# probabilists/zuko

Hardware: AMD Instinct MI355X
Metric: log_prob samples/sec, NSF d=64 K=8 bins=8 batch=2^20 (higher is better)
Workload: dtype f32; 1 GPU; NSF(features=64, context=0, transforms=8, bins=8, hidden=[256]*3) log_prob, batch=2^20 per GPU, x~N(0,1), seed-0 init; batch_per_gpu=1048576, global_batch=1048576, parallelism=batch-sharded x1, one RCCL all-reduce of the scalar NLL

## Files before the change

zuko_amd/csrc/fused_ar_half_impl.h:

```cpp
#pragma once
#include "fused_ar_split_impl.h"

#ifndef ARH_LOOK
#define ARH_LOOK 1
#endif
#ifndef ARH_RELU_INT
#define ARH_RELU_INT 0
#endif
#ifndef ARH_EPI_PINNED
#define ARH_EPI_PINNED 1
#endif
#ifndef ARH_DESCALE_PK
#define ARH_DESCALE_PK 1
#endif
#ifndef ARH_PREFETCH
#define ARH_PREFETCH 1
#endif
#ifndef ARH_BLOCK_ASM
#define ARH_BLOCK_ASM 1
#endif
#ifndef ARH_EPI_TILE
#define ARH_EPI_TILE 1
#endif

#ifndef ARH_SPLIT_GAPS
#define ARH_SPLIT_GAPS 1
#endif

namespace zk {

typedef _Float16 f16x8 __attribute__((ext_vector_type(8)));

struct ArhB {
  f16x8 h, l;
};

__device__ __forceinline__ void arh_scale(float& amax, float& s, float& inv_s) {
  amax = fmaxf(amax, __shfl_xor(amax, 16, 64));
  amax = fmaxf(amax, __shfl_xor(amax, 32, 64));
  int e = __builtin_amdgcn_frexp_expf(amax);
  int ea = 15 - e;
  ea = ea > 90 ? 90 : (ea < -90 ? -90 : ea);
  s = __builtin_amdgcn_ldexpf(1.0f, ea);
  inv_s = __builtin_amdgcn_ldexpf(1.0f, -ea);
}

#define ARH_AMAX_OVERFLOW (65520.f * 0x1p90f)

typedef unsigned arh_u32x4 __attribute__((ext_vector_type(4)));
typedef float arh_f32x2 __attribute__((ext_vector_type(2)));

__device__ __forceinline__ void arh_split(const f32x4& lo, const f32x4& hi, float s, ArhB& b) {
  if (ARX_ABL == 6) {
    b.h = __builtin_bit_cast(f16x8, lo); b.l = __builtin_bit_cast(f16x8, hi);
    return;
  }
#if ARH_EPI_PINNED
  const float nz = -0.f;
  unsigned h0, h1, h2, h3, l0, l1, l2, l3;
#define ARH_SPLIT_H(OP, H, V) "v_fma_mix" OP "_f16 %[" H "], %[" V "], %[s], %[nz]\n\t"
#define ARH_SPLIT_L(OP, SEL, L, H, V) "v_fma_mix" OP "_f16 %[" L "], %[" V "], %[s], -%[" H "] op_sel:[0,0," SEL "] op_sel_hi:[0,0,1]\n\t"
  asm(ARH_SPLIT_H("lo", "h0", "v0") ARH_SPLIT_H("lo", "h1", "v2") ARH_SPLIT_H("lo", "h2", "v4") ARH_SPLIT_H("lo", "h3", "v6")
      ARH_SPLIT_H("hi", "h0", "v1") ARH_SPLIT_H("hi", "h1", "v3") ARH_SPLIT_H("hi", "h2", "v5") ARH_SPLIT_H("hi", "h3", "v7")
      ARH_SPLIT_L("lo", "0", "l0", "h0", "v0") ARH_SPLIT_L("lo", "0", "l1", "h1", "v2") ARH_SPLIT_L("lo", "0", "l2", "h2", "v4") ARH_SPLIT_L("lo", "0", "l3", "h3", "v6")
      ARH_SPLIT_L("hi", "1", "l0", "h0", "v1") ARH_SPLIT_L("hi", "1", "l1", "h1", "v3") ARH_SPLIT_L("hi", "1", "l2", "h2", "v5") ARH_SPLIT_L("hi", "1", "l3", "h3", "v7")
      : [h0] "=&v"(h0), [h1] "=&v"(h1), [h2] "=&v"(h2), [h3] "=&v"(h3), [l0] "=&v"(l0), [l1] "=&v"(l1), [l2] "=&v"(l2), [l3] "=&v"(l3)
      : [v0] "v"(lo[0]), [v1] "v"(lo[1]), [v2] "v"(lo[2]), [v3] "v"(lo[3]), [v4] "v"(hi[0]), [v5] "v"(hi[1]), [v6] "v"(hi[2]), [v7] "v"(hi[3]), [s] "v"(s), [nz] "s"(nz));
#undef ARH_SPLIT_H
#undef ARH_SPLIT_L
  b.h = __builtin_bit_cast(f16x8, arh_u32x4{h0, h1, h2, h3}); b.l = __builtin_bit_cast(f16x8, arh_u32x4{l0, l1, l2, l3});
  return;
#endif
#pragma unroll
  for (int e = 0; e < 8; ++e) {
    const float v = (e < 4 ? lo[e] : hi[e - 4]) * s;
    const _Float16 h = (_Float16)v;
    const float r = v - (float)h;
    b.h[e] = h;
    b.l[e] = (_Float16)r;
  }
}

#define ARH_MFMA(A, B, C) C = __builtin_amdgcn_mfma_f32_16x16x32_f16(__builtin_bit_cast(f16x8, A), B, C, 0, 0, 0)
__device__ __forceinline__ void arh_block(const f32x4 (&a)[2], const ArhB& b, f32x4& c) {
  if (ARX_ABL == 2) {
    asm volatile("" ::"v"(a[0]), "v"(a[1]));
    return;
  }
  ARH_MFMA(a[1], b.h, c);
  ARH_MFMA(a[0], b.l, c);
  ARH_MFMA(a[0], b.h, c);
}

__device__ __forceinline__ void arh_touch(f32x4& v) { asm volatile("" : "+v"(v)); }
template <int N> __device__ __forceinline__ void arh_settle(f32x4& a0, f32x4& a1) { asm volatile("s_waitcnt lgkmcnt(%2)" : "+v"(a0), "+v"(a1) : "n"(N)); }
template <int N> __device__ __forceinline__ void arh_settle(f32x4& a0, f32x4& a1, f32x4& a2) { asm volatile("s_waitcnt lgkmcnt(%3)" : "+v"(a0), "+v"(a1), "+v"(a2) : "n"(N)); }

constexpr bool ARH_BLK = ARH_BLOCK_ASM && ARX_ABL != 2;
constexpr bool ARH_GAPS = ARH_SPLIT_GAPS && ARH_BLK && ARH_EPI_PINNED && ARX_ABL != 6;
struct ArhHL {
  unsigned h0, h1, h2, h3, l0, l1, l2, l3;
};
#define ARH_GH(OP, H, V) "\n\tv_fma_mix" OP "_f16 %[" H "], %[" V "], %[s], %[nz]"
#define ARH_GL(OP, SEL, L, H, V) "\n\tv_fma_mix" OP "_f16 %[" L "], %[" V "], %[s], -%[" H "] op_sel:[0,0," SEL "] op_sel_hi:[0,0,1]"
#define ARH_G0 ARH_GH("lo", "h0", "v0")
#define ARH_G1 ARH_GH("lo", "h1", "v2")
#define ARH_G2 ARH_GH("lo", "h2", "v4")
#define ARH_G3 ARH_GH("lo", "h3", "v6")
#define ARH_G4 ARH_GH("hi", "h0", "v1")
#define ARH_G5 ARH_GH("hi", "h1", "v3")
#define ARH_G6 ARH_GH("hi", "h2", "v5")
#define ARH_G7 ARH_GH("hi", "h3", "v7")
#define ARH_G8 ARH_GL("lo", "0", "l0", "h0", "v0")
#define ARH_G9 ARH_GL("lo", "0", "l1", "h1", "v2")
#define ARH_G10 ARH_GL("lo", "0", "l2", "h2", "v4")
#define ARH_G11 ARH_GL("lo", "0", "l3", "h3", "v6")
#define ARH_G12 ARH_GL("hi", "1", "l0", "h0", "v1")
#define ARH_G13 ARH_GL("hi", "1", "l1", "h1", "v3")
#define ARH_G14 ARH_GL("hi", "1", "l2", "h2", "v5")
#define ARH_G15 ARH_GL("hi", "1", "l3", "h3", "v7")
#define ARH_G_OUT0
#define ARH_G_IN0
#define ARH_G_SC [s] "v"(s), [nz] "s"(nz)
#define ARH_G_OUT1 , [h0] "=&v"(x.h0), [l0] "=&v"(x.l0)
#define ARH_G_IN1 , [v0] "v"(lo[0]), [v1] "v"(lo[1]), ARH_G_SC
#define ARH_G_OUT2 , [l0] "+v"(x.l0), [h1] "=&v"(x.h1)
#define ARH_G_IN2 , [v1] "v"(lo[1]), [h0] "v"(x.h0), [v2] "v"(lo[2]), [v3] "v"(lo[3]), ARH_G_SC
#define ARH_G_OUT3 , [l1] "=&v"(x.l1), [h2] "=&v"(x.h2)
#define ARH_G_IN3 , [v2] "v"(lo[2]), [v3] "v"(lo[3]), [h1] "v"(x.h1), [v4] "v"(hi[0]), ARH_G_SC
#define ARH_G_OUT4 , [h2] "+v"(x.h2), [l2] "=&v"(x.l2)
#define ARH_G_IN4 , [v5] "v"(hi[1]), [v4] "v"(hi[0]), ARH_G_SC
#define ARH_G_OUT5 , [h3] "=&v"(x.h3), [l3] "=&v"(x.l3)
#define ARH_G_IN5 , [v6] "v"(hi[2]), [v7] "v"(hi[3]), ARH_G_SC
#define ARH_G_OUT6 , [l3] "+v"(x.l3)
#define ARH_G_IN6 , [v7] "v"(hi[3]), [h3] "v"(x.h3), [s] "v"(s)
#define ARH_T_OUT2 [l0] "+v"(x.l0), [h1] "=&v"(x.h1), [l1] "=&v"(x.l1), [h2] "=&v"(x.h2), [l2] "=&v"(x.l2), [h3] "=&v"(x.h3), [l3] "=&v"(x.l3)
#define ARH_T_IN2 [v1] "v"(lo[1]), [v2] "v"(lo[2]), [v3] "v"(lo[3]), [v4] "v"(hi[0]), [v5] "v"(hi[1]), [v6] "v"(hi[2]), [v7] "v"(hi[3]), [h0] "v"(x.h0), ARH_G_SC
#define ARH_T_OUT3 [l1] "=&v"(x.l1), [h2] "=&v"(x.h2), [l2] "=&v"(x.l2), [h3] "=&v"(x.h3), [l3] "=&v"(x.l3)
#define ARH_T_IN3 [v2] "v"(lo[2]), [v3] "v"(lo[3]), [v4] "v"(hi[0]), [v5] "v"(hi[1]), [v6] "v"(hi[2]), [v7] "v"(hi[3]), [h1] "v"(x.h1), ARH_G_SC
#define ARH_T_OUT4 [h2] "+v"(x.h2), [l2] "=&v"(x.l2), [h3] "=&v"(x.h3), [l3] "=&v"(x.l3)
#define ARH_T_IN4 [v4] "v"(hi[0]), [v5] "v"(hi[1]), [v6] "v"(hi[2]), [v7] "v"(hi[3]), ARH_G_SC
#define ARH_T_OUT5 [h3] "=&v"(x.h3), [l3] "=&v"(x.l3)
#define ARH_T_IN5 [v6] "v"(hi[2]), [v7] "v"(hi[3]), ARH_G_SC
#define ARH_T_OUT6 [l3] "+v"(x.l3)
#define ARH_T_IN6 [v7] "v"(hi[3]), [h3] "v"(x.h3), [s] "v"(s)
#define ARH_BLK_ASM(C0, COUT, POST, BSOUT, G1, G2, G3, G)                                                   \
  asm volatile("v_mfma_f32_16x16x32_f16 %[c], %[al], %[bh], " C0 G1 "\n\t"                                  \
               "v_mfma_f32_16x16x32_f16 %[c], %[ah], %[bl], %[c]" G2 "\n\t"                                 \
               "v_mfma_f32_16x16x32_f16 %[c], %[ah], %[bh], %[c]" G3 POST                                   \
               : [c] COUT(c) ARH_BLK_BS##BSOUT ARH_G_OUT##G                                                 \
               : [ah] "v"(a[0]), [al] "v"(a[1]), [bh] "v"(b.h), [bl] "v"(b.l) ARH_G_IN##G)
#define ARH_BLK_BS0
#define ARH_BLK_BS1 , "+v"(bs)
#define ARH_BLK_FORM(G1, G2, G3, G)                                                               \
  if constexpr (FIRST && TILE) ARH_BLK_ASM("0", "=&v", "\n\ts_nop 11", 1, G1, G2, G3, G);          \
  else if constexpr (FIRST) ARH_BLK_ASM("0", "=&v", "", 0, G1, G2, G3, G);                         \
  else if constexpr (TILE) ARH_BLK_ASM("%[c]", "+v", "\n\ts_nop 11", 1, G1, G2, G3, G);            \
  else ARH_BLK_ASM("%[c]", "+v", "", 0, G1, G2, G3, G)
template <int N, bool FIRST, bool PAD, bool TILE> __device__ __forceinline__ void arh_wait_block(f32x4 (&a)[2], const ArhB& b, f32x4& c, f32x4& bs) {
  static_assert(N >= 0 && N < 16, "lgkmcnt is a four-bit field");
  if constexpr (PAD) asm volatile("s_nop 0");
  __builtin_amdgcn_s_waitcnt(0xC07F | (N << 8));
  if (ARX_FENCE) __builtin_amdgcn_sched_barrier(0);
  ARH_BLK_FORM("", "", "", 0);
  if (ARX_FENCE) __builtin_amdgcn_sched_barrier(0);
}
template <int N, bool FIRST, bool PAD, bool TILE, int GF>
__device__ __forceinline__ void arh_wait_block(f32x4 (&a)[2], const ArhB& b, f32x4& c, f32x4& bs, ArhHL& x, const f32x4& lo, const f32x4& hi, float s) {
  static_assert(N >= 0 && N < 16 && GF >= 1 && GF <= 6, "lgkmcnt is a four-bit field; six forms");
  const float nz = -0.f;
  if constexpr (PAD) asm volatile("s_nop 0");
  __builtin_amdgcn_s_waitcnt(0xC07F | (N << 8));
  if (ARX_FENCE) __builtin_amdgcn_sched_barrier(0);
  if constexpr (GF == 1) { ARH_BLK_FORM(ARH_G0, ARH_G4, ARH_G8, 1); }
  else if constexpr (GF == 2) { ARH_BLK_FORM(ARH_G12, ARH_G1, ARH_G5, 2); }
  else if constexpr (GF == 3) { ARH_BLK_FORM(ARH_G9, ARH_G13, ARH_G2, 3); }
  else if constexpr (GF == 4) { ARH_BLK_FORM(ARH_G6, ARH_G10, ARH_G14, 4); }
  else if constexpr (GF == 5) { ARH_BLK_FORM(ARH_G3, ARH_G7, ARH_G11, 5); }
  else { ARH_BLK_FORM(ARH_G15, "", "", 6); }
  if (ARX_FENCE) __builtin_amdgcn_sched_barrier(0);
}
template <int F> __device__ __forceinline__ void arh_split_tail(ArhHL& x, const f32x4& lo, const f32x4& hi, float s) {
  static_assert(F >= 2 && F <= 6, "six forms");
  const float nz = -0.f;
#define ARH_T6 ARH_G15
#define ARH_T5 ARH_G3 ARH_G7 ARH_G11 ARH_T6
#define ARH_T4 ARH_G6 ARH_G10 ARH_G14 ARH_T5
#define ARH_T3 ARH_G9 ARH_G13 ARH_G2 ARH_T4
#define ARH_T2 ARH_G12 ARH_G1 ARH_G5 ARH_T3
#define ARH_TAIL_ASM(T, F) asm("; the rest of a split" T : ARH_T_OUT##F : ARH_T_IN##F)
  if constexpr (F == 2) ARH_TAIL_ASM(ARH_T2, 2);
  else if constexpr (F == 3) ARH_TAIL_ASM(ARH_T3, 3);
  else if constexpr (F == 4) ARH_TAIL_ASM(ARH_T4, 4);
  else if constexpr (F == 5) ARH_TAIL_ASM(ARH_T5, 5);
  else ARH_TAIL_ASM(ARH_T6, 6);
#undef ARH_TAIL_ASM
#undef ARH_T2
#undef ARH_T3
#undef ARH_T4
#undef ARH_T5
#undef ARH_T6
}
__device__ __forceinline__ void arh_split_done(const ArhHL& x, ArhB& b) {
  b.h = __builtin_bit_cast(f16x8, arh_u32x4{x.h0, x.h1, x.h2, x.h3}); b.l = __builtin_bit_cast(f16x8, arh_u32x4{x.l0, x.l1, x.l2, x.l3});
  asm volatile("" : "+v"(b.h), "+v"(b.l));
}
#undef ARH_BLK_FORM
#undef ARH_BLK_ASM
#undef ARH_BLK_BS0
#undef ARH_BLK_BS1
#undef ARH_G_OUT0
#undef ARH_G_IN0
#undef ARH_G_OUT1
#undef ARH_G_IN1
#undef ARH_G_OUT2
#undef ARH_G_IN2
#undef ARH_G_OUT3
#undef ARH_G_IN3
#undef ARH_G_OUT4
#undef ARH_G_IN4
#undef ARH_G_OUT5
#undef ARH_G_IN5
#undef ARH_G_OUT6
#undef ARH_G_IN6
#undef ARH_G_SC
#undef ARH_T_OUT2
#undef ARH_T_IN2
#undef ARH_T_OUT3
#undef ARH_T_IN3
#undef ARH_T_OUT4
#undef ARH_T_IN4
#undef ARH_T_OUT5
#undef ARH_T_IN5
#undef ARH_T_OUT6
#undef ARH_T_IN6
#undef ARH_GH
#undef ARH_GL
#undef ARH_G0
#undef ARH_G1
#undef ARH_G2
#undef ARH_G3
#undef ARH_G4
#undef ARH_G5
#undef ARH_G6
#undef ARH_G7
#undef ARH_G8
#undef ARH_G9
#undef ARH_G10
#undef ARH_G11
#undef ARH_G12
#undef ARH_G13
#undef ARH_G14
#undef ARH_G15
template <int NT> __device__ __forceinline__ void arh_acc_ready(f32x4 (&acc)[NT]) {
  asm volatile("s_nop 11" : "+v"(acc[NT - 1]));
#pragma unroll
  for (int t = 0; t + 1 < NT; ++t) arh_touch(acc[t]);
}

__device__ __forceinline__ void arh_relu_max(f32x4& o, float (&pm)[4], int t) {
#pragma unroll
  for (int r = 0; r < 4; r += 2)
    asm("v_max_f32 %0, 0, %0\n\tv_max_f32 %1, 0, %1\n\tv_max3_f32 %2, %2, %0, %1" : "+v"(o[r]), "+v"(o[r + 1]), "+v"(pm[(2 * t + r / 2) % 4]));
}
__device__ __forceinline__ float arh_join_max(const float (&pm)[4]) {
  float amax;
  asm("v_max_f32 %0, %1, %2\n\tv_max3_f32 %0, %0, %3, %4" : "=&v"(amax) : "v"(pm[0]), "v"(pm[1]), "v"(pm[2]), "v"(pm[3]));
  return amax;
}

template <int WAVES, int CH, int NR> struct ArhRing : ArRingS<WAVES, CH, NR> {
  typedef ArRingS<WAVES, CH, NR> B;
  template <int XV> __device__ __forceinline__ void advance_x() {
    asm volatile("s_waitcnt vmcnt(%0) lgkmcnt(0)" ::"n"((NR - 2) * B::PER + XV) : "memory");
    if (ARX_ABL != 4) __builtin_amdgcn_s_barrier();
    asm volatile("" ::: "memory");
    this->issue();
    this->slot = (this->slot + 1 == NR) ? 0 : this->slot + 1;
    this->cur_off = this->lds_off + (unsigned)(this->slot * CH * AR_TF * 4 + this->lane * 16);
  }
  template <int S, int XV = 0> __device__ __forceinline__ f32x4 read() {
    if constexpr (XV != 0 && S % CH == 0) {
      advance_x<XV>();
      f32x4 v;
      if (ARX_ABL == 5) {
        asm volatile("v_mov_b32 %0, %1" : "=v"(v[0]) : "v"(this->cur_off));
        v[1] = v[2] = v[3] = v[0];
        return v;
      }
      asm volatile("ds_read_b128 %0, %1 offset:%2" : "=v"(v) : "v"(this->cur_off), "n"((S % CH) * AR_TF * 4));
      return v;
    } else {
      return B::template read<S>();
    }
  }
};

template <int WAVES, int CH, int IMAGES, int BPOS, bool FLOW = false> struct ArhRing4 {
  static constexpr int NR = 4, PER = CH / WAVES, PIVOT = PER > 4 ? 4 : 0, CHB = CH * AR_TF * 4, NCH = (IMAGES + CH - 1) / CH;
  static_assert(PER * WAVES == CH && PER <= 6 && BPOS % 2 == 0 && BPOS >= 2 * (ARH_LOOK + 1) && BPOS + 1 < CH && CH % 2 == 0 && IMAGES % 2 == 0, "ring geometry");
  static constexpr int trigger(int c) {
    const int last = (IMAGES < (c + 1) * CH ? IMAGES : (c + 1) * CH) - 1;
    return c * CH + BPOS + 1 < last ? c * CH + BPOS + 1 : last;
  }
  static constexpr int first_trigger_from(int pos) {
    for (int c = 0; c < NCH; ++c)
      if (trigger(c) >= pos) return trigger(c);
    return -1;
  }
  const char* gsrc;
  char* ldst;
  unsigned goff, gend;
  unsigned fill_off;
  unsigned read_off;
  unsigned lane_off;
  unsigned lane16;
  unsigned cur_off;
  bool rows_in_flight;
  const char* bias_src;
  char* bias_dst;
  int bias_n, wave_id;
  __device__ __forceinline__ void bias_request() {
    for (int p = wave_id; p < bias_n; p += WAVES)
      __builtin_amdgcn_global_load_lds((const __attribute__((address_space(1))) void*)(bias_src + p * 1024 + (size_t)lane16), (__attribute__((address_space(3))) void*)(bias_dst + p * 1024), 16, 0, 0);
  }
  __device__ __forceinline__ void start(float* lds, const float* stream, int n_chunks, int wave, int lane) {
    const int b0 = wave * PER + PIVOT;
    gsrc = reinterpret_cast<const char*>(stream + b0 * AR_TF);
    ldst = reinterpret_cast<char*>(lds + b0 * AR_TF);
    goff = 0; gend = (unsigned)n_chunks * CHB; fill_off = 0;
    lane16 = (unsigned)lane * 16;
    lane_off = (unsigned)(size_t)((__attribute__((address_space(3))) float*)lds) + lane16;
    if constexpr (FLOW) { wave_id = wave; rows_in_flight = false; bias_n = 0; }
#pragma unroll
    for (int i = 0; i < NR - 1; ++i) issue();
    read_off = (NR - 1) * CHB;
    cur_off = lane_off;
  }
  template <int I> __device__ __forceinline__ void dma(const char* g, char* l) {
    if constexpr (I < PER) {
      __builtin_amdgcn_global_load_lds((const __attribute__((address_space(1))) void*)g, (__attribute__((address_space(3))) void*)l, 16, (I - PIVOT) * AR_TF * 4, 0);
      dma<I + 1>(g, l);
    }
  }
  __device__ __forceinline__ void issue() {
    asm volatile("" : "+v"(lane16));
    if (ARX_ABL != 1) dma<0>(gsrc + goff + (size_t)lane16, ldst + fill_off);
    goff = (goff + CHB == gend) ? 0 : goff + CHB;
    fill_off = (fill_off + CHB == NR * CHB) ? 0 : fill_off + CHB;
  }
  template <int XV, bool DRAIN> __device__ __forceinline__ void wait() {
    if constexpr (DRAIN) asm volatile("s_waitcnt vmcnt(%0) lgkmcnt(0)" ::"n"(XV) : "memory");
    else asm volatile("s_waitcnt vmcnt(%0)" ::"n"(XV) : "memory");
  }
  template <int XV, bool DRAIN> __device__ __forceinline__ void boundary() {
    if constexpr (FLOW && XV != 0) {
      if (rows_in_flight) wait<XV, DRAIN>();
      else wait<0, DRAIN>();
    } else {
      wait<XV, DRAIN>();
    }
    if (ARX_ABL != 4) __builtin_amdgcn_s_barrier();
    asm volatile("" ::: "memory");
    issue();
    asm volatile("" ::: "memory");
  }
  template <int S, int XV = 0> __device__ __forceinline__ f32x4 read() {
    static_assert(S >= 0 && S < IMAGES, "stream position");
    if constexpr (S % CH == 0) {
      read_off = (read_off + CHB == NR * CHB) ? 0 : read_off + CHB;
      cur_off = lane_off + read_off;
    }
    f32x4 v;
    if (ARX_ABL == 5) {
      asm volatile("v_mov_b32 %0, %1" : "=v"(v[0]) : "v"(cur_off));
      v[1] = v[2] = v[3] = v[0];
    } else {
      asm volatile("ds_read_b128 %0, %1 offset:%2" : "=v"(v) : "v"(cur_off), "n"((S % CH) * AR_TF * 4));
    }
    if constexpr (S == trigger(S / CH)) boundary<XV, (S % CH != BPOS + 1)>();
    if constexpr (FLOW && NCH >= 2) {
      if constexpr (S == trigger(NCH - 2)) bias_request();
    }
    return v;
  }
};

template <class S, int L, bool ALT> constexpr int arh_ip(int s) {
  if constexpr (ALT) return S::B_IP_ALT[s];
  else return ArxPat<S>::ip(L, s);
}
template <class S> constexpr bool ARH_EPI = S::ACT == 1 && ARH_EPI_PINNED && ARH_EPI_TILE;

template <int NBLK> struct ArhGapPlan {
  signed char pair[NBLK > 0 ? NBLK : 1], form[NBLK > 0 ? NBLK : 1];
  short lim[9];
  signed char front[9];
};
template <class S, int L, int NT> constexpr int arh_gap_blocks() {
  if constexpr (L == S::NH) return S::GOFF[S::NG] * NT;
  else return S::NB[L];
}
template <class S, int L, int NT> constexpr int arh_gap_reader(int b) {
  if constexpr (L == S::NH) return S::G_IP[b / NT];
  else return ArxPat<S>::ip(L, b);
}
template <class S, int L> constexpr int arh_gap_last_block(int t) {
  if (t >= S::HT[L]) return S::NB[L];
  int last = -1;
  for (int b = 0; b < S::NB[L]; ++b)
    if (ArxPat<S>::ot(L, b) == t) last = b;
  return last;
}
template <class S, int L, int NT> constexpr ArhGapPlan<arh_gap_blocks<S, L, NT>()> arh_gap_plan() {
  static_assert(L >= 1 && L <= S::NH && S::TMAX / 2 <= 8, "a consuming layer; eight in pairs at most");
  constexpr int NBLK = arh_gap_blocks<S, L, NT>(), NP = (S::HT[L - 1] + 1) / 2;
  ArhGapPlan<NBLK> g{};
  for (int p = 0; p < 9; ++p) { g.lim[p] = 0; g.front[p] = 7; }
  int cursor = 0;
  for (int p = 1; p < NP; ++p) {
    int lim = NBLK;
    for (int b = NBLK - 1; b >= 0; --b)
      if (arh_gap_reader<S, L, NT>(b) == p) lim = b;
    if constexpr (L != S::NH) {
      for (int t = 2 * p; t <= 2 * p + 1; ++t) {
        const int last = arh_gap_last_block<S, L>(t);
        lim = last < 0 ? 0 : (last < lim ? last : lim);
      }
    }
    int f = 1;
    for (; f <= 6 && cursor < lim; ++f, ++cursor) { g.pair[cursor] = (signed char)p; g.form[cursor] = (signed char)f; }
    g.lim[p] = (short)lim;
    g.front[p] = (signed char)f;
  }
  return g;
}
template <class S, int L, int NT, bool ON> struct ArhGapsOf {
  static constexpr int NP = 0, NBLK = 0;
  static constexpr int form(int) { return 0; }
  static constexpr int pair(int) { return 0; }
  static constexpr bool tail_at(int, int) { return false; }
  static constexpr bool any_tail_at(int) { return false; }
  static constexpr int front(int) { return 7; }
};
template <class S, int L, int NT> struct ArhGapsOf<S, L, NT, true> {
  static constexpr int NP = (S::HT[L - 1] + 1) / 2, NBLK = arh_gap_blocks<S, L, NT>();
  static constexpr ArhGapPlan<NBLK> plan = arh_gap_plan<S, L, NT>();
  static constexpr int form(int b) { return plan.form[b]; }
  static constexpr int pair(int b) { return plan.pair[b]; }
  static constexpr bool tail_at(int p, int b) { return p >= 1 && plan.front[p] <= 6 && plan.lim[p] == b; }
  static constexpr int front(int p) { return plan.front[p]; }
  static constexpr bool any_tail_at(int b) {
    for (int p = 1; p < NP; ++p)
      if (tail_at(p, b)) return true;
    return false;
  }
};
template <class GP, int HTI, int NPR> __device__ __forceinline__ void arh_gap_front(const f32x4 (&out)[2 * NPR], float s, ArhB (&in)[NPR]) {
  const f32x4 zero = {0.f, 0.f, 0.f, 0.f};
  arh_split(out[0], 1 < HTI ? out[1] : zero, s, in[0]);
  ars_for<GP::NP>([&](auto p_) ARS_ALWAYS_INLINE {
    constexpr int p = p_;
    if constexpr (GP::tail_at(p, 0)) arh_split(out[2 * p], 2 * p + 1 < HTI ? out[2 * p + 1] : zero, s, in[p]);
  });
}
template <class GP, int HTI, int B, int NPR> __device__ __forceinline__ void arh_gap_tails(ArhHL (&x)[NPR], const f32x4 (&out)[2 * NPR], float s, ArhB (&in)[NPR]) {
  const f32x4 zero = {0.f, 0.f, 0.f, 0.f};
  ars_for<GP::NP>([&](auto p_) ARS_ALWAYS_INLINE {
    constexpr int p = p_;
    if constexpr (B >= 1 && GP::tail_at(p, B)) {
      if constexpr (GP::front(p) == 1) {
        arh_split(out[2 * p], 2 * p + 1 < HTI ? out[2 * p + 1] : zero, s, in[p]);
      } else {
        arh_split_tail<GP::front(p)>(x[p], out[2 * p], 2 * p + 1 < HTI ? out[2 * p + 1] : zero, s);
        arh_split_done(x[p], in[p]);
      }
    }
  });
}

template <class S, int L, class Ring, bool ALT = false, bool GAPS = false>
__device__ __forceinline__ void arh_hidden(Ring& ring, const float* bias_q, ArhB (&in)[S::TMAX / 2], f32x4 (&out)[S::TMAX], float d, float (&pm)[4], float s_in = 0.f) {
  typedef ArxPat<S> P;
  typedef ArhGapsOf<S, L, 0, GAPS> GP;
  constexpr int NB = S::NB[L], BASE = S::BASE[L], HTL = S::HT[L], HTI = S::HT[L > 0 ? L - 1 : 0];
  ArhHL x[S::TMAX / 2];
  const f32x4 zero = {0.f, 0.f, 0.f, 0.f};
  if constexpr (GAPS) arh_gap_front<GP, HTI>(out, s_in, in);
  ars_for<HTL>([&](auto t_) ARS_ALWAYS_INLINE {
    constexpr int t = t_;
    if constexpr (!P::tile_has_blocks(L, t)) {
      out[t] = *reinterpret_cast<const f32x4*>(bias_q + t * 16);
      if constexpr (ARH_EPI<S>) arh_relu_max(out[t], pm, t);
    }
  });
  if constexpr (NB > 0) {
    constexpr int LOOK = ARH_LOOK < NB ? ARH_LOOK : NB;
    f32x4 a[LOOK + 1][2];
    f32x4 bs;
    f32x4 acc;
    const unsigned bias_addr = arx_lds_addr(bias_q);
    ars_for<LOOK>([&](auto b_) ARS_ALWAYS_INLINE {
      constexpr int b = b_;
      ars_for<2>([&](auto p) ARS_ALWAYS_INLINE { a[b][p] = ring.template read<BASE + 2 * b + decltype(p)::value>(); });
    });
    ars_for<NB>([&](auto s_) ARS_ALWAYS_INLINE {
      constexpr int s = s_, ot = P::ot(L, s), cur = s % (LOOK + 1);
      constexpr int ip = arh_ip<S, L, ALT>(s);
      constexpr bool first_of_tile = (s == 0 || P::ot(L, s - 1) != ot), last_of_tile = (s + 1 == NB || P::ot(L, s + 1) != ot);
      if constexpr (first_of_tile && !ARH_BLK) acc = f32x4{0.f, 0.f, 0.f, 0.f};
      if constexpr (last_of_tile) bs = arx_lds_raw<ot * 64>(bias_addr);
      if constexpr (s + LOOK < NB) {
        constexpr int nx = (s + LOOK) % (LOOK + 1);
        ars_for<2>([&](auto p) ARS_ALWAYS_INLINE { a[nx][p] = ring.template read<BASE + 2 * (s + LOOK) + decltype(p)::value>(); });
      }
      constexpr int ahead = (s + LOOK < NB ? LOOK : NB - 1 - s);
      if constexpr (GAPS) arh_gap_tails<GP, HTI, s>(x, out, s_in, in);
      constexpr int WAIT = last_of_tile ? (s + LOOK < NB ? 2 : 0) : 2 * ahead;
      constexpr bool pad = s == 0 || (GAPS && s >= 1 && GP::any_tail_at(s));
      if constexpr (GP::form(s) != 0) {
        constexpr int gp = GP::pair(s);
        arh_wait_block<WAIT, first_of_tile, pad, last_of_tile, GP::form(s)>(a[cur], in[ip], acc, bs, x[gp], out[2 * gp], 2 * gp + 1 < HTI ? out[2 * gp + 1] : zero, s_in);
        if constexpr (GP::form(s) == 6) arh_split_done(x[gp], in[gp]);
      } else if constexpr (ARH_BLK) {
        arh_wait_block<WAIT, first_of_tile, pad, last_of_tile>(a[cur], in[ip], acc, bs);
      } else {
        if constexpr (last_of_tile) arh_settle<(s + LOOK < NB ? 2 : 0)>(a[cur][0], a[cur][1], bs);
        else arh_settle<2 * ahead>(a[cur][0], a[cur][1]);
        if (ARX_FENCE) __builtin_amdgcn_sched_barrier(0);
        arh_block(a[cur], in[ip], acc);
        if (ARX_FENCE) __builtin_amdgcn_sched_barrier(0);
      }
      if constexpr (last_of_tile) {
        if (ARH_DESCALE_PK) {
#pragma unroll
          for (int r = 0; r < 4; r += 2) {
            const arh_f32x2 o = __builtin_elementwise_fma(arh_f32x2{acc[r], acc[r + 1]}, arh_f32x2{d, d}, arh_f32x2{bs[r], bs[r + 1]});
            out[ot][r] = o[0]; out[ot][r + 1] = o[1];
          }
        } else {
#pragma unroll
          for (int r = 0; r < 4; ++r) out[ot][r] = __builtin_fmaf(acc[r], d, bs[r]);
        }
        if constexpr (ARH_EPI<S>) arh_relu_max(out[ot], pm, ot);
      }
    });
    if constexpr (GAPS) arh_gap_tails<GP, HTI, NB>(x, out, s_in, in);
  }
}

template <class S, int L, class Ring, bool HAS_ALT = false> __device__ __forceinline__ void arh_hidden_stack(Ring& ring, const float* bias_lds, int q, ArhB (&in)[S::TMAX / 2], f32x4 (&out)[S::TMAX], const float* wd,
                                                                                                         float& inv_s, float& poison, float& s, bool alt = false) {
  if constexpr (L < S::NH) {
    float pm[4] = {0.f, 0.f, 0.f, 0.f};
    if constexpr (HAS_ALT && L == 0) {
      static_assert(S::BASE[0] == 0, "B_IP_ALT lists the first layer's blocks");
      if (alt) arh_hidden<S, L, Ring, true>(ring, bias_lds + L * S::BIAS_STRIDE + 4 * q, in, out, wd[L] * inv_s, pm);
      else arh_hidden<S, L, Ring>(ring, bias_lds + L * S::BIAS_STRIDE + 4 * q, in, out, wd[L] * inv_s, pm);
    } else {
      arh_hidden<S, L, Ring, false, ARH_GAPS && L >= 1>(ring, bias_lds + L * S::BIAS_STRIDE + 4 * q, in, out, wd[L] * inv_s, pm, s);
    }
    constexpr int HTL = S::HT[L];
    float amax = 0.f;
    if constexpr (S::ACT == 1 && ARH_EPI_PINNED) {
      if constexpr (!ARH_EPI_TILE) {
#pragma unroll
        for (int t = 0; t < HTL; ++t) arh_relu_max(out[t], pm, t);
      }
      amax = arh_join_max(pm);
    } else if constexpr (S::ACT == 1) {
#pragma unroll
      for (int t = 0; t < HTL; ++t)
#pragma unroll
        for (int r = 0; r < 4; ++r) {
          if (ARH_RELU_INT) out[t][r] = __builtin_bit_cast(float, max(__builtin_bit_cast(int, out[t][r]), 0));
          else out[t][r] = out[t][r] < 0.f ? 0.f : out[t][r];
          amax = fmaxf(amax, out[t][r]);
        }
    } else {
      ar_activate<S::ACT, HTL>(out, out);
#pragma unroll
      for (int t = 0; t < HTL; ++t)
#pragma unroll
        for (int r = 0; r < 4; ++r) amax = fmaxf(amax, fabsf(out[t][r]));
    }
    arh_scale(amax, s, inv_s);
    if constexpr (S::ACT == 1 && ARH_EPI_PINNED) {
      if (!(amax < ARH_AMAX_OVERFLOW)) poison = __builtin_nanf("");
    }
    if constexpr (!ARH_GAPS) {
      const f32x4 zero = {0.f, 0.f, 0.f, 0.f};
#pragma unroll
      for (int p = 0; p < (HTL + 1) / 2; ++p) arh_split(out[2 * p], 2 * p + 1 < HTL ? out[2 * p + 1] : zero, s, in[p]);
    }
    arh_hidden_stack<S, L + 1, Ring, HAS_ALT>(ring, bias_lds, q, in, out, wd, inv_s, poison, s, alt);
  }
}

template <typename Uni> __device__ __forceinline__ void arh_flow_epilogue(float (&p)[4 * Uni::NT], const ArArgs& a, const int (&fid)[Uni::FPL], const float (&xin)[Uni::FPL], float poison, float* xr,
                                                                          const float* base, int D, bool term, float& lacc) {
  constexpr int FPL = Uni::FPL, TOTAL = Uni::TOTAL;
#pragma unroll
  for (int fi = 0; fi < FPL; ++fi) Uni::template poison<false>(p, fi * TOTAL, poison);
  auto ld = [&](int i) { return p[i]; };
#pragma unroll
  for (int fi = 0; fi < FPL; ++fi) {
    const int f = fid[fi];
    if (f >= 0) {
      float yv, lj;
      Uni::fwd(ld, fi * TOTAL, a, xin[fi], yv, lj);
      lacc += lj;
      if (term) {
        const float df = yv - base[f];
        lacc += __builtin_fmaf(-(df * df), base[D + f], base[2 * D + f]);
      } else {
        xr[f] = yv;
      }
    }
  }
}

template <class S, typename Uni, bool DIAG, bool TERM, bool FLOW, class Ring, class XReq, class Fids>
__device__ __forceinline__ void arh_pass(const ArArgs& a, Ring& ring, XReq& x_request, f32x4 (&xnext)[S::NIT], float* bias_lds, const Fids& fids, float* xr, const float* base, const ArLane& ln,
                                         int64_t tile, const float* wd, bool first, bool last, bool term, float& total, bool alt = false) {
  constexpr bool RING4 = S::NR == 4;
  static_assert(!FLOW || (RING4 && S::XLDS && S::DIN == S::D && !DIAG && !TERM), "flow pass: four-slot ring, rows in LDS, no context columns");
  constexpr int NT = Uni::NT, FPL = Uni::FPL, WAVES = S::WAVES;
  constexpr int NG = S::NG;
  constexpr int NSTEP = S::GOFF[NG];
  constexpr bool XLDS = S::XLDS;
  const int wave = ln.wave, j = ln.j, q = ln.q;
  const float* bias_last = bias_lds + S::NH * S::BIAS_STRIDE;
  const unsigned bias_last_addr = arx_lds_addr(bias_last + 4 * q);
  if constexpr (FLOW) {
    asm volatile("" ::: "memory");
    __builtin_amdgcn_wave_barrier();
  }
  const int64_t n = tile * (16 * WAVES) + wave * 16 + j;
  const bool live = n < a.N;
  const int64_t nc = live ? n : a.N - 1;
  const float* xrow = a.x + nc * a.ldx;

  ArhB in[S::TMAX / 2];
  f32x4 out[S::TMAX];
  float poison;
  float inv_s;
  {
    f32x4 xin[S::NIT + 1];
#pragma unroll
    for (int it = 0; it < S::NIT; ++it) {
      f32x4 v = {0.f, 0.f, 0.f, 0.f};
      if constexpr (FLOW) {
        if ((it + 1) * 16 <= S::DIN || it * 16 + 4 * q < S::DIN) v = *reinterpret_cast<const f32x4*>(xr + it * 16 + 4 * q);
      } else if (ARH_PREFETCH) {
        if ((it + 1) * 16 <= S::DIN || it * 16 + 4 * q < S::DIN) v = xnext[it];
      } else {
        if ((it + 1) * 16 <= S::DIN || it * 16 + 4 * q < S::DIN) v = *reinterpret_cast<const f32x4*>(xrow + it * 16 + 4 * q);
      }
      xin[it] = v;
    }
    xin[S::NIT] = f32x4{0.f, 0.f, 0.f, 0.f};
    poison = ar_poison_of<S::NIT>(xin);
    float amax = 0.f;
#pragma unroll
    for (int it = 0; it < S::NIT; ++it)
#pragma unroll
      for (int r = 0; r < 4; ++r) amax = fmaxf(amax, fabsf(xin[it][r]));
    if constexpr (XLDS && !FLOW) ar_rows_in<S::D>(xr, q, xin);
    float s;
    arh_scale(amax, s, inv_s);
    if constexpr (S::ACT == 1 && ARH_EPI_PINNED) {
      if (!(amax < ARH_AMAX_OVERFLOW)) poison = __builtin_nanf("");
    }
#pragma unroll
    for (int p = 0; p < (S::NIT + 1) / 2; ++p) arh_split(xin[2 * p], xin[2 * p + 1], s, in[p]);
  }

  float ladj_in = 0.f;
  if constexpr (!FLOW) {
    if (ARH_PREFETCH && a.ladj && a.accumulate && live && q == 0) ladj_in = a.ladj[n];
  }

  float s_last = 0.f;
  if constexpr (FLOW) arh_hidden_stack<S, 0, Ring, S::FLOW_ALT>(ring, bias_lds, q, in, out, wd, inv_s, poison, s_last, alt);
  else arh_hidden_stack<S, 0, Ring>(ring, bias_lds, q, in, out, wd, inv_s, poison, s_last);
  typedef ArhGapsOf<S, S::NH, Uni::NT, (ARH_GAPS && S::NH >= 1)> GP;
  constexpr int HTI = S::HT[S::NH >= 1 ? S::NH - 1 : 0];
  ArhHL hl[S::TMAX / 2];
  const f32x4 zero = {0.f, 0.f, 0.f, 0.f};
  if constexpr (ARH_GAPS && S::NH >= 1) arh_gap_front<GP, HTI>(out, s_last, in);

  const float dl = wd[S::NH] * inv_s;
  float lacc = 0.f;
  constexpr int NBL = NSTEP * NT;
  constexpr int LOOKL = ARH_LOOK < NBL ? ARH_LOOK : NBL;
  f32x4 w[LOOKL + 1][2];
  constexpr int XPOS = []() constexpr {
    if constexpr (!ARH_PREFETCH) return -1;
    else if constexpr (RING4) return Ring::first_trigger_from(S::LAST_BASE);
    else return (S::LAST_BASE + S::CH - 1) / S::CH * S::CH;
  }();
  if constexpr (FLOW) {
    asm volatile("" ::: "memory");
    if (last) {
      x_request(tile + gridDim.x < a.n_tiles ? tile + gridDim.x : tile, xnext);
    } else {
#pragma unroll
      for (int it = 0; it < S::NIT; ++it) asm("" : "=v"(xnext[it]));
    }
    ring.rows_in_flight = last;
    asm volatile("" ::: "memory");
  } else if (ARH_PREFETCH) {
    asm volatile("" ::: "memory");
    x_request(tile + gridDim.x < a.n_tiles ? tile + gridDim.x : tile, xnext);
    asm volatile("" ::: "memory");
  }
#define ARH_READ_LAST(POS) ring.template read<(POS), ((POS) == XPOS ? S::NIT : 0)>()
  ars_for<LOOKL>([&](auto b_) ARS_ALWAYS_INLINE {
    constexpr int b = b_;
    ars_for<2>([&](auto p) ARS_ALWAYS_INLINE { w[b][p] = ARH_READ_LAST(S::LAST_BASE + 2 * b + decltype(p)::value); });
  });
  ars_for<NG>([&](auto g_) ARS_ALWAYS_INLINE {
    constexpr int g = g_, ST0 = S::GOFF[g], GN = S::GOFF[g + 1] - S::GOFF[g];
    int fid[FPL];
    float xin[FPL];
    fids.template fetch<XLDS>(g, xr, xrow, fid, xin);
    float bv[3 * FPL];
    if constexpr (TERM && !FLOW) fids.fetch_base(fid, base, S::D, bv);
    f32x4 acc[NT], bs[NT];
    if constexpr (GN == 0) {
      const float* bg = bias_last + (g * NT) * 16 + 4 * q;
      ars_for<NT>([&](auto t) ARS_ALWAYS_INLINE { bs[t] = *reinterpret_cast<const f32x4*>(bg + t * 16); });
    }
    if constexpr (GN == 0 || !ARH_BLK) ars_for<NT>([&](auto t) ARS_ALWAYS_INLINE { acc[t] = f32x4{0.f, 0.f, 0.f, 0.f}; });
    ars_for<GN>([&](auto i_) ARS_ALWAYS_INLINE {
      constexpr int st = ST0 + decltype(i_)::value, ip = S::G_IP[st];
      ars_for<NT>([&](auto t_) ARS_ALWAYS_INLINE {
        constexpr int t = t_, blk = st * NT + t, cur = blk % (LOOKL + 1);
        constexpr bool last_of_group = (decltype(i_)::value == GN - 1 && t == NT - 1);
        if constexpr (last_of_group) {
          ars_for<NT>([&](auto u) ARS_ALWAYS_INLINE { bs[u] = arx_lds_raw<(g * NT + decltype(u)::value) * 64>(bias_last_addr); });
        }
        if constexpr (blk + LOOKL < NBL) {
          constexpr int nx = (blk + LOOKL) % (LOOKL + 1);
          ars_for<2>([&](auto p) ARS_ALWAYS_INLINE { w[nx][p] = ARH_READ_LAST(S::LAST_BASE + 2 * (blk + LOOKL) + decltype(p)::value); });
        }
        constexpr int ahead = (blk + LOOKL < NBL ? LOOKL : NBL - 1 - blk);
        if constexpr (ARH_GAPS && S::NH >= 1) arh_gap_tails<GP, HTI, blk>(hl, out, s_last, in);
        constexpr int WAIT = last_of_group ? (blk + LOOKL < NBL ? 2 : 0) : 2 * ahead;
        constexpr bool pad = blk == 0 || (ARH_GAPS && S::NH >= 1 && blk >= 1 && GP::any_tail_at(blk));
        if constexpr (ARH_BLK) {
          if constexpr (GP::form(blk) != 0) {
            constexpr int gp = GP::pair(blk);
            arh_wait_block<WAIT, decltype(i_)::value == 0, pad, false, GP::form(blk)>(w[cur], in[ip], acc[t], bs[0], hl[gp], out[2 * gp], 2 * gp + 1 < HTI ? out[2 * gp + 1] : zero, s_last);
            if constexpr (GP::form(blk) == 6) arh_split_done(hl[gp], in[gp]);
          } else {
            arh_wait_block<WAIT, decltype(i_)::value == 0, pad, false>(w[cur], in[ip], acc[t], bs[0]);
          }
          if constexpr (last_of_group) {
#pragma unroll
            for (int u = 0; u < NT; ++u) arh_touch(bs[u]);
            arh_acc_ready<NT>(acc);
          }
        } else {
          if constexpr (last_of_group) arh_settle<(blk + LOOKL < NBL ? 2 : 0)>(w[cur][0], w[cur][1]);
          else arh_settle<2 * ahead>(w[cur][0], w[cur][1]);
          if constexpr (last_of_group) {
#pragma unroll
            for (int u = 0; u < NT; ++u) arh_touch(bs[u]);
          }
          if (ARX_FENCE) __builtin_amdgcn_sched_barrier(0);
          arh_block(w[cur], in[ip], acc[t]);
          if (ARX_FENCE) __builtin_amdgcn_sched_barrier(0);
        }
      });
    });
    float p[4 * NT];
    ars_for<NT>([&](auto t) ARS_ALWAYS_INLINE {
#pragma unroll
      for (int r = 0; r < 4; ++r) {
        p[4 * t + r] = __builtin_fmaf(acc[t][r], dl, bs[t][r]);
        if (ARH_POISON_ONE) asm("" : "+v"(p[4 * t + r]));
      }
    });
    if constexpr (FLOW) arh_flow_epilogue<Uni>(p, a, fid, xin, poison, xr, base, S::D, last && term, lacc);
    else ar_uni_epilogue<Uni, DIAG, XLDS, true, TERM>(p, a, fid, xin, poison, xr, n, live, S::D, lacc, bv);
  });
#undef ARH_READ_LAST
  if constexpr (ARH_GAPS && S::NH >= 1) arh_gap_tails<GP, HTI, NBL>(hl, out, s_last, in);
  if constexpr (FLOW) {
    lacc += __shfl_xor(lacc, 16, 64);
    lacc += __shfl_xor(lacc, 32, 64);
    total = first ? lacc : total + lacc;
    if (last) {
      if (live && q == 0) a.ladj[n] = total;
      if (!term) ar_rows_out<S::D>(xr, q, a.y + n * a.ldy, live);
    }
    return;
  }
  if (ARH_PREFETCH) ar_ladj_store<true>(a, lacc, n, live, q, ladj_in);
  if constexpr (XLDS && !TERM) ar_rows_out<S::D>(xr, q, a.y + n * a.ldy, live);
  if (!ARH_PREFETCH) ar_ladj_store(a, lacc, n, live, q);
}

template <class S, typename Uni, bool DIAG, bool TERM> __device__ __forceinline__ void arh_body(const ArArgs& a) {
  constexpr bool RING4 = S::NR == 4;
  typedef std::conditional_t<RING4, ArhRing4<S::WAVES, S::CH, S::IMAGES, S::BPOS>, ArhRing<S::WAVES, S::CH, S::NR>> Ring;
  static_assert(S::WAVES == 8 && (S::NR == 3 || S::NR == 4) && S::TMAX <= 16 && S::TMAX % 2 == 0 && S::OCC == 2, "two-part split kernels: widths <= 256, two wavefronts per SIMD");
  constexpr int NT = Uni::NT, FPL = Uni::FPL, WAVES = S::WAVES;
  constexpr int NG = S::NG;
  constexpr int NSTEP = S::GOFF[NG];
  static_assert(S::IMAGES == S::LAST_BASE + 2 * NSTEP * NT && (S::IMAGES + S::CH - 1) / S::CH == S::NCHUNK, "stream length");
  const ArLane ln;
  const int tid = ln.tid, lane = ln.lane, wave = ln.wave, j = ln.j, q = ln.q;

  Ring ring;
  if constexpr (RING4) {
    ring.start(ars_lds, a.stream, a.n_chunks, wave, lane);
  } else {
    ring.lds = ars_lds; ring.stream = a.stream; ring.n_chunks = a.n_chunks; ring.wave = wave; ring.lane = lane;
    ring.load_chunk = 0; ring.load_slot = 0;
#pragma unroll
    for (int i = 0; i < S::NR - 1; ++i) ring.issue();
    ring.slot = S::NR - 1;
    ring.lds_off = (unsigned)(size_t)((__attribute__((address_space(3))) float*)ars_lds);
    ring.cur_off = ring.lds_off;
  }

  auto x_request = [&](int64_t tile, f32x4 (&xv)[S::NIT]) ARS_ALWAYS_INLINE {
    const int64_t n = tile * (16 * WAVES) + wave * 16 + j;
    const float* row = a.x + (n < a.N ? n : a.N - 1) * a.ldx;
#pragma unroll
    for (int it = 0; it < S::NIT; ++it) {
      const int col = it * 16 + 4 * q;
      xv[it] = *reinterpret_cast<const f32x4*>(row + ((it + 1) * 16 <= S::DIN || col < S::DIN ? col : S::DIN - 4));
    }
  };
  f32x4 xnext[S::NIT];
  if (ARH_PREFETCH) x_request(blockIdx.x, xnext);

  float* const bias_lds = ars_lds + S::NR * S::CH * AR_TF;
  int* const fmap_lds = ArLds::fmap(bias_lds, a.bias_floats);
  float* const xr = ArLds::row(fmap_lds, wave, j, a.xs);
  float* const base = ArLds::base(fmap_lds, NG * 4 * FPL);
  if constexpr (TERM) ArLds::stage_base<64 * WAVES>(a, tid, base, S::D);
  ArLds::stage<64 * WAVES>(a, tid, bias_lds, fmap_lds, NG * 4 * FPL);
// ... 127 lines not shown
```

Before: 77.55 million samples/s.

## Defer tile descale and ReLU epilogue into the next tile's MFMA gaps

Double-buffers the accumulator and bias registers so that a tile's descale FMA and ReLU/max epilogue can be deferred past the end of its last MFMA block. The ReLU and running-max instructions are emitted inside a later block's inline-asm MFMA sequence, filling the dependency gaps between MFMAs. The s_nop 11 drain is only kept on tiles that still end immediately. This aims to hide epilogue VALU latency and nop stalls behind matrix work, at the cost of more live VGPRs and a complex constexpr schedule whose correctness relies on static_asserts.

Result: no change. 78.24 million samples/s, median of 6 (+0.9%).

```diff
diff --git a/zuko_amd/csrc/fused_ar_half_impl.h b/zuko_amd/csrc/fused_ar_half_impl.h
--- a/zuko_amd/csrc/fused_ar_half_impl.h
+++ b/zuko_amd/csrc/fused_ar_half_impl.h
@@ -25,6 +25,9 @@
 
 #ifndef ARH_SPLIT_GAPS
 #define ARH_SPLIT_GAPS 1
+#endif
+#ifndef ARH_EPI_GAPS
+#define ARH_EPI_GAPS 1
 #endif
 
 namespace zk {
@@ -152,12 +155,35 @@
                : [ah] "v"(a[0]), [al] "v"(a[1]), [bh] "v"(b.h), [bl] "v"(b.l) ARH_G_IN##G)
 #define ARH_BLK_BS0
 #define ARH_BLK_BS1 , "+v"(bs)
+#define ARH_BLK_NOP(C0, COUT, BSOUT, G1, G2, G3, G)                                               \
+  if constexpr (NOPK == 11) ARH_BLK_ASM(C0, COUT, "\n\ts_nop 11", BSOUT, G1, G2, G3, G);          \
+  else if constexpr (NOPK == 1) ARH_BLK_ASM(C0, COUT, "\n\ts_nop 1", BSOUT, G1, G2, G3, G);       \
+  else ARH_BLK_ASM(C0, COUT, "", BSOUT, G1, G2, G3, G)
 #define ARH_BLK_FORM(G1, G2, G3, G)                                                               \
-  if constexpr (FIRST && TILE) ARH_BLK_ASM("0", "=&v", "\n\ts_nop 11", 1, G1, G2, G3, G);          \
-  else if constexpr (FIRST) ARH_BLK_ASM("0", "=&v", "", 0, G1, G2, G3, G);                         \
-  else if constexpr (TILE) ARH_BLK_ASM("%[c]", "+v", "\n\ts_nop 11", 1, G1, G2, G3, G);            \
-  else ARH_BLK_ASM("%[c]", "+v", "", 0, G1, G2, G3, G)
-template <int N, bool FIRST, bool PAD, bool TILE> __device__ __forceinline__ void arh_wait_block(f32x4 (&a)[2], const ArhB& b, f32x4& c, f32x4& bs) {
+  if constexpr (FIRST && TILE) { ARH_BLK_NOP("0", "=&v", 1, G1, G2, G3, G); }                      \
+  else if constexpr (FIRST) { ARH_BLK_NOP("0", "=&v", 0, G1, G2, G3, G); }                         \
+  else if constexpr (TILE) { ARH_BLK_NOP("%[c]", "+v", 1, G1, G2, G3, G); }                        \
+  else { ARH_BLK_NOP("%[c]", "+v", 0, G1, G2, G3, G); }
+#define ARH_E1 "\n\tv_max_f32 %[o0], 0, %[o0]\n\tv_max_f32 %[o1], 0, %[o1]"
+#define ARH_E2 "\n\tv_max_f32 %[o2], 0, %[o2]\n\tv_max_f32 %[o3], 0, %[o3]"
+#define ARH_E3 "\n\tv_max3_f32 %[pa], %[pa], %[o0], %[o1]\n\tv_max3_f32 %[pb], %[pb], %[o2], %[o3]"
+#define ARH_G_OUTE , [o0] "+v"(o[0]), [o1] "+v"(o[1]), [o2] "+v"(o[2]), [o3] "+v"(o[3]), [pa] "+v"(pa), [pb] "+v"(pb)
+#define ARH_G_INE
+template <int N, bool FIRST, bool PAD, bool TILE, int NOPK>
+__device__ __forceinline__ void arh_wait_block_epi(f32x4 (&a)[2], const ArhB& b, f32x4& c, f32x4& bs, f32x4& o, float& pa, float& pb) {
+  static_assert(N >= 0 && N < 16, "lgkmcnt is a four-bit field");
+  if constexpr (PAD) asm volatile("s_nop 0");
+  __builtin_amdgcn_s_waitcnt(0xC07F | (N << 8));
+  if (ARX_FENCE) __builtin_amdgcn_sched_barrier(0);
+  ARH_BLK_FORM(ARH_E1, ARH_E2, ARH_E3, E);
+  if (ARX_FENCE) __builtin_amdgcn_sched_barrier(0);
+}
+#undef ARH_E1
+#undef ARH_E2
+#undef ARH_E3
+#undef ARH_G_OUTE
+#undef ARH_G_INE
+template <int N, bool FIRST, bool PAD, bool TILE, int NOPK = (TILE ? 11 : 0)> __device__ __forceinline__ void arh_wait_block(f32x4 (&a)[2], const ArhB& b, f32x4& c, f32x4& bs) {
   static_assert(N >= 0 && N < 16, "lgkmcnt is a four-bit field");
   if constexpr (PAD) asm volatile("s_nop 0");
   __builtin_amdgcn_s_waitcnt(0xC07F | (N << 8));
@@ -165,7 +191,7 @@
   ARH_BLK_FORM("", "", "", 0);
   if (ARX_FENCE) __builtin_amdgcn_sched_barrier(0);
 }
-template <int N, bool FIRST, bool PAD, bool TILE, int GF>
+template <int N, bool FIRST, bool PAD, bool TILE, int GF, int NOPK = (TILE ? 11 : 0)>
 __device__ __forceinline__ void arh_wait_block(f32x4 (&a)[2], const ArhB& b, f32x4& c, f32x4& bs, ArhHL& x, const f32x4& lo, const f32x4& hi, float s) {
   static_assert(N >= 0 && N < 16 && GF >= 1 && GF <= 6, "lgkmcnt is a four-bit field; six forms");
   const float nz = -0.f;
@@ -206,6 +232,7 @@
   asm volatile("" : "+v"(b.h), "+v"(b.l));
 }
 #undef ARH_BLK_FORM
+#undef ARH_BLK_NOP
 #undef ARH_BLK_ASM
 #undef ARH_BLK_BS0
 #undef ARH_BLK_BS1
@@ -479,6 +506,71 @@
   });
 }
 
+struct ArhEpiPlan {
+  short db[16], ub[16];
+};
+template <class S, int L, class GP> constexpr ArhEpiPlan arh_epi_plan() {
+  typedef ArxPat<S> P;
+  constexpr int NB = S::NB[L], HTL = S::HT[L];
+  static_assert(HTL <= 16, "sixteen out tiles at most");
+  ArhEpiPlan e{};
+  for (int t = 0; t < 16; ++t) e.db[t] = e.ub[t] = -1;
+  int cursor = 0;
+  for (int t = 0; t + 1 < HTL; ++t) {
+    if (arh_gap_last_block<S, L>(t) < 0) continue;
+    int n = -1;
+    for (int u = HTL - 1; u > t; --u)
+      if (arh_gap_last_block<S, L>(u) >= 0) n = u;
+    if (n < 0) continue;
+    int db = NB;
+    for (int b = NB - 1; b >= 0; --b)
+      if (P::ot(L, b) == n) db = b;
+    int ub = -1;
+    for (int b = db + 1 > cursor ? db + 1 : cursor; b < NB && ub < 0; ++b)
+      if (GP::form(b) == 0 && P::ot(L, b - 1) == P::ot(L, b)) ub = b;
+    if (ub < 0) continue;
+    e.db[t] = (short)db; e.ub[t] = (short)ub;
+    cursor = ub + 1;
+  }
+  return e;
+}
+template <class S, int L, class GP> constexpr bool arh_epi_ok(const ArhEpiPlan& e) {
+  for (int t = 0; t < S::HT[L]; ++t) {
+    if (e.db[t] < 0) continue;
+    if (e.db[t] != arh_gap_last_block<S, L>(t) + 1 || e.ub[t] <= e.db[t] || e.ub[t] >= S::NB[L]) return false;
+    for (int b = e.db[t]; b < S::NB[L]; ++b)
+      if (GP::form(b) != 0 && GP::pair(b) == t / 2) return false;
+  }
+  return true;
+}
+template <class S, int L, class GP, bool ON> struct ArhEpiOf {
+  static constexpr int slot(int) { return 0; }
+  static constexpr bool deferred(int) { return false; }
+  static constexpr int db_tile(int) { return -1; }
+  static constexpr int ub_tile(int) { return -1; }
+};
+template <class S, int L, class GP> struct ArhEpiOf<S, L, GP, true> {
+  static constexpr ArhEpiPlan plan = arh_epi_plan<S, L, GP>();
+  static_assert(arh_epi_ok<S, L, GP>(plan), "a deferred descale in front of a split form that reads its tile, or blocks of a tile apart");
+  static constexpr int slot(int t) {
+    int k = 0;
+    for (int u = 0; u < t; ++u)
+      if (arh_gap_last_block<S, L>(u) >= 0) k ^= 1;
+    return k;
+  }
+  static constexpr bool deferred(int t) { return plan.db[t] >= 0; }
+  static constexpr int db_tile(int b) {
+    for (int t = 0; t < S::HT[L]; ++t)
+      if (plan.db[t] == b) return t;
+    return -1;
+  }
+  static constexpr int ub_tile(int b) {
+    for (int t = 0; t < S::HT[L]; ++t)
+      if (plan.ub[t] == b) return t;
+    return -1;
+  }
+};
+
 template <class S, int L, class Ring, bool ALT = false, bool GAPS = false>
 __device__ __forceinline__ void arh_hidden(Ring& ring, const float* bias_q, ArhB (&in)[S::TMAX / 2], f32x4 (&out)[S::TMAX], float d, float (&pm)[4], float s_in = 0.f) {
   typedef ArxPat<S> P;
@@ -497,8 +589,21 @@
   if constexpr (NB > 0) {
     constexpr int LOOK = ARH_LOOK < NB ? ARH_LOOK : NB;
     f32x4 a[LOOK + 1][2];
-    f32x4 bs;
-    f32x4 acc;
+    typedef ArhEpiOf<S, L, GP, (ARH_EPI_GAPS && ARH_BLK && ARH_EPI<S>)> EP;
+    f32x4 bs[2];
+    f32x4 acc[2];
+    auto descale = [&](f32x4& o, const f32x4& c, const f32x4& bias) ARS_ALWAYS_INLINE {
+      if (ARH_DESCALE_PK) {
+#pragma unroll
+        for (int r = 0; r < 4; r += 2) {
+          const arh_f32x2 v = __builtin_elementwise_fma(arh_f32x2{c[r], c[r + 1]}, arh_f32x2{d, d}, arh_f32x2{bias[r], bias[r + 1]});
+          o[r] = v[0]; o[r + 1] = v[1];
+        }
+      } else {
+#pragma unroll
+        for (int r = 0; r < 4; ++r) o[r] = __builtin_fmaf(c[r], d, bias[r]);
+      }
+    };
     const unsigned bias_addr = arx_lds_addr(bias_q);
     ars_for<LOOK>([&](auto b_) ARS_ALWAYS_INLINE {
       constexpr int b = b_;
@@ -508,8 +613,12 @@
       constexpr int s = s_, ot = P::ot(L, s), cur = s % (LOOK + 1);
       constexpr int ip = arh_ip<S, L, ALT>(s);
       constexpr bool first_of_tile = (s == 0 || P::ot(L, s - 1) != ot), last_of_tile = (s + 1 == NB || P::ot(L, s + 1) != ot);
-      if constexpr (first_of_tile && !ARH_BLK) acc = f32x4{0.f, 0.f, 0.f, 0.f};
-      if constexpr (last_of_tile) bs = arx_lds_raw<ot * 64>(bias_addr);
+      constexpr int k = EP::slot(ot), dt = EP::db_tile(s), ut = EP::ub_tile(s);
+      constexpr bool ends = last_of_tile && !EP::deferred(ot);
+      constexpr int NOPK = ends ? 11 : (dt >= 0 && (GP::form(s) == 0 || GP::form(s) == 6) ? 1 : 0);
+      static_assert((dt < 0 || (first_of_tile && EP::slot(dt) == (k ^ 1))) && (ut < 0 || GP::form(s) == 0), "arh_epi_plan");
+      if constexpr (first_of_tile && !ARH_BLK) acc[k] = f32x4{0.f, 0.f, 0.f, 0.f};
+      if constexpr (last_of_tile) bs[k] = arx_lds_raw<ot * 64>(bias_addr);
       if constexpr (s + LOOK < NB) {
         constexpr int nx = (s + LOOK) % (LOOK + 1);
         ars_for<2>([&](auto p) ARS_ALWAYS_INLINE { a[nx][p] = ring.template read<BASE + 2 * (s + LOOK) + decltype(p)::value>(); });
@@ -520,28 +629,22 @@
       constexpr bool pad = s == 0 || (GAPS && s >= 1 && GP::any_tail_at(s));
       if constexpr (GP::form(s) != 0) {
         constexpr int gp = GP::pair(s);
-        arh_wait_block<WAIT, first_of_tile, pad, last_of_tile, GP::form(s)>(a[cur], in[ip], acc, bs, x[gp], out[2 * gp], 2 * gp + 1 < HTI ? out[2 * gp + 1] : zero, s_in);
+        arh_wait_block<WAIT, first_of_tile, pad, last_of_tile, GP::form(s), NOPK>(a[cur], in[ip], acc[k], bs[k], x[gp], out[2 * gp], 2 * gp + 1 < HTI ? out[2 * gp + 1] : zero, s_in);
         if constexpr (GP::form(s) == 6) arh_split_done(x[gp], in[gp]);
+      } else if constexpr (ARH_BLK && ut >= 0) {
+        arh_wait_block_epi<WAIT, first_of_tile, pad, last_of_tile, NOPK>(a[cur], in[ip], acc[k], bs[k], out[ut], pm[(2 * ut) % 4], pm[(2 * ut + 1) % 4]);
       } else if constexpr (ARH_BLK) {
-        arh_wait_block<WAIT, first_of_tile, pad, last_of_tile>(a[cur], in[ip], acc, bs);
+        arh_wait_block<WAIT, first_of_tile, pad, last_of_tile, NOPK>(a[cur], in[ip], acc[k], bs[k]);
       } else {
-        if constexpr (last_of_tile) arh_settle<(s + LOOK < NB ? 2 : 0)>(a[cur][0], a[cur][1], bs);
+        if constexpr (last_of_tile) arh_settle<(s + LOOK < NB ? 2 : 0)>(a[cur][0], a[cur][1], bs[k]);
         else arh_settle<2 * ahead>(a[cur][0], a[cur][1]);
         if (ARX_FENCE) __builtin_amdgcn_sched_barrier(0);
-        arh_block(a[cur], in[ip], acc);
+        arh_block(a[cur], in[ip], acc[k]);
         if (ARX_FENCE) __builtin_amdgcn_sched_barrier(0);
       }
-      if constexpr (last_of_tile) {
-        if (ARH_DESCALE_PK) {
-#pragma unroll
-          for (int r = 0; r < 4; r += 2) {
-            const arh_f32x2 o = __builtin_elementwise_fma(arh_f32x2{acc[r], acc[r + 1]}, arh_f32x2{d, d}, arh_f32x2{bs[r], bs[r + 1]});
-            out[ot][r] = o[0]; out[ot][r + 1] = o[1];
-          }
-        } else {
-#pragma unroll
-          for (int r = 0; r < 4; ++r) out[ot][r] = __builtin_fmaf(acc[r], d, bs[r]);
-        }
+      if constexpr (dt >= 0) descale(out[dt], acc[k ^ 1], bs[k ^ 1]);
+      if constexpr (ends) {
+        descale(out[ot], acc[k], bs[k]);
         if constexpr (ARH_EPI<S>) arh_relu_max(out[ot], pm, ot);
       }
     });
```
